# KhutornoyYaroslav/vcm-ts

Hardware: AMD Instinct MI355X
Metric: encoded frames/sec at 1920x1080 GOP-32 (higher is better)
Workload: dtype f32 (fp16x3 split-MFMA, fp32 accumulate)

## Files before the change

### include/dcvc_hip.h

```cpp
#ifndef DCVC_HIP_H
#define DCVC_HIP_H

#include <stdint.h>

#ifdef __cplusplus
extern "C" {
#endif

#define DCVC_OK 0
#define DCVC_E_ARG (-1)
#define DCVC_E_LAUNCH (-2)
#define DCVC_E_RANGE (-3)

#define DCVC_STATUS_ACT_SATURATED 1

#define DCVC_MAX_SEG 3

#define DCVC_PREC_FP32 0
#define DCVC_PREC_FP16X3 1

typedef struct {
    const float *ptr;
    int32_t C;
    int32_t cs;
// ... 1 lines not shown

typedef struct {
    dcvc_seg seg[DCVC_MAX_SEG];
    int32_t nseg;
    int32_t N, Hin, Win;
    int32_t in_act;
    float in_slope;
    const float *wpack;
    const float *bpack;
    int32_t ks;
    int32_t stride;
    int32_t Cout;
    int32_t Cout_pad;
    float *out;
    int32_t out_cs;
    int32_t out_act;
    float out_slope;
    int32_t pixel_shuffle;
    const float *res;
    int32_t res_cs;
    const float *res_gate;
    const float *res2;
    int32_t res2_cs;
    int32_t precision;
    int32_t *status;
    float *chan_partial;
    int32_t tile_row0;
    int32_t tile_rows;
    int32_t pair_taps;
} dcvc_conv_args;

int32_t dcvc_conv_tile_rows(int32_t ks, int32_t stride);

int32_t dcvc_conv_chan_partial_parts(int32_t ks, int32_t stride, int32_t Hout, int32_t Wout);
int dcvc_channel_mean_finish(const float *chan_partial, int32_t parts, int32_t row_stride, float *mean, int32_t N,
                             int32_t C, int32_t HW, void *stream);

int64_t dcvc_conv_pack_size(int32_t Cout, int32_t ks, int32_t nseg, const int32_t *seg_C, int32_t *cout_pad);

int dcvc_conv_pack_weights(const float *w, const float *b, int32_t Cout, int32_t ks, int32_t nseg,
                           const int32_t *seg_C, int32_t pixel_shuffle, int32_t precision, float *wpack,
                           float *bpack);

int64_t dcvc_conv_pack_size_paired(int32_t Cout, int32_t Cin, int32_t *cout_pad);
int dcvc_conv_pack_weights_paired(const float *w, const float *b, int32_t Cout, int32_t Cin, float *wpack, float *bpack);

int dcvc_conv2d(const dcvc_conv_args *a, void *stream);
int dcvc_conv_set_lookahead(int32_t mode);

int64_t dcvc_conv_small_pack_bytes(int32_t Cout, int32_t ks, int32_t nseg, const int32_t *seg_C);
int dcvc_conv_small_pack_weights(const float *w, const float *b, int32_t Cout, int32_t ks, int32_t nseg,
                                 const int32_t *seg_C, void *wpack, float *bpack);
int dcvc_conv2d_small(const dcvc_conv_args *a, void *stream);

int64_t dcvc_conv_k32_pack_bytes(int32_t Cout, int32_t ks, int32_t nseg, const int32_t *seg_C, int32_t *cout_pad);
int dcvc_conv_k32_pack_weights(const float *w, const float *b, int32_t Cout, int32_t ks, int32_t nseg,
                               const int32_t *seg_C, int32_t pixel_shuffle, void *wpack, float *bpack);
int dcvc_conv2d_k32(const dcvc_conv_args *a, void *stream);
int dcvc_conv_k32_set_waves(int32_t waves);

int dcvc_warp(const float *src, int32_t src_cs, const float *flow, int32_t flow_cs, float *out, int32_t out_cs,
              int32_t N, int32_t H, int32_t W, int32_t C, void *stream);
int dcvc_up2(const float *src, int32_t src_cs, float *out, int32_t out_cs, float *out2, int32_t out2_cs,
             int32_t N, int32_t H, int32_t W, int32_t C, float scale, void *stream);
int dcvc_down2(const float *src, int32_t src_cs, float *out, int32_t out_cs, int32_t N, int32_t H, int32_t W,
               int32_t C, float scale, int32_t avgpool_order, void *stream);
int dcvc_maxpool2(const float *src, int32_t src_cs, float *out, int32_t out_cs, int32_t N, int32_t H, int32_t W,
                  int32_t C, void *stream);
int dcvc_copy_channels(const float *src, int32_t src_cs, float *out, int32_t out_cs, int64_t npix, int32_t C,
                       void *stream);
int dcvc_nchw_to_nhwc(const float *src, float *out, int32_t out_cs, int32_t N, int32_t C, int32_t H, int32_t W,
                      void *stream);
int dcvc_nhwc_to_nchw(const float *src, int32_t src_cs, float *out, int32_t N, int32_t C, int32_t H, int32_t W,
                      int32_t clamp01, void *stream);

int dcvc_channel_mean(const float *src, int32_t src_cs, float *mean, float *scratch, int32_t N, int32_t HW,
                      int32_t C, void *stream);
int dcvc_se_gate(const float *mean, const float *w1, const float *w2, float *gate, int32_t N, int32_t C,
                 int32_t Cr, void *stream);

int dcvc_scale_channels(const float *src, int32_t src_cs, float *out, int32_t out_cs, const float *q_basic,
                        const float *q_scale, int32_t mode, int32_t N, int32_t HW, int32_t C, void *stream);
int dcvc_scale_channels_map(const float *src, int32_t src_cs, float *out, int32_t out_cs, const float *q_basic,
                            const float *q_scale, int32_t mode, int32_t N, int32_t HW, int32_t C, const float *q_map,
                            int32_t H, int32_t W, void *stream);
int dcvc_round_symbols(const float *z, int32_t z_cs, float *z_hat, int32_t zh_cs, int32_t *sym, int32_t N,
                       int32_t H, int32_t W, int32_t C, void *stream);
int dcvc_symbols_to_nhwc(const int32_t *sym, float *out, int32_t out_cs, int32_t N, int32_t H, int32_t W,
                         int32_t C, void *stream);

typedef struct {
    const float *y;
    int32_t y_cs;
    const float *fusion;
    int32_t fusion_cs;
    const float *spatial;
    int32_t spatial_cs;
    float *params;
    int32_t params_cs;
    float *y_hat;
    float *y_q;
    float *y_res;
    float *scales_hat;
    int32_t *sym;
    int32_t *idx;
    float *out;
// ... 35 lines not shown
```

### vcm_ts_amd/csrc/conv_small.hip

```cpp
#include <hip/hip_runtime.h>
#include <stdint.h>
#include <string.h>

#include "dcvc_hip.h"
#include "kernel_common.h"

namespace {

constexpr int KC = 16;

struct SmallK {
    const float *seg_ptr[DCVC_MAX_SEG];
    int seg_C[DCVC_MAX_SEG];
    int seg_cs[DCVC_MAX_SEG];
    int nseg;
    int H, W;
    int in_act;
    float in_slope;
    const char *wpack;
    const float *bpack;
    int Cout;
    float *out;
    int out_cs, out_act;
    float out_slope;
    const float *res;
    int res_cs;
    int *status;
};

template <int KS>
__global__ __launch_bounds__(256, 3) void conv_small(const SmallK a) {
    constexpr int RPW = 2, BH = 4 * RPW, BW = 32, PAD = KS / 2, PH = BH + KS - 1, PW = BW + KS - 1, T = KS * KS;
    constexpr int TPS = KS, NST = KS;
    constexpr int PATCH_F = PH * PW * 16;
    constexpr int SLAB_F = TPS * 4 * 16 * 4;
    __shared__ __attribute__((aligned(16))) float lds[PATCH_F + SLAB_F];
    char *patch = (char *)lds;
    float *wl = lds + PATCH_F;

    const int tid = threadIdx.x, lane = tid & 63, wave = tid >> 6;
    const int x0 = blockIdx.x * BW, y0 = blockIdx.y * BH, img = blockIdx.z;
    const int pr = lane & 15, g = lane >> 4;

    f32x4 acc[RPW][2];
#pragma unroll
    for (int m = 0; m < RPW; ++m)
#pragma unroll
        for (int hf = 0; hf < 2; ++hf) acc[m][hf] = (f32x4){0.f, 0.f, 0.f, 0.f};

    constexpr int NP = (PH * PW * 4 + 255) / 256, NW = (SLAB_F / 4 + 255) / 256;
    f32x4 rp[NP], rw[NW];
    struct Cursor {
        int s, c0, cg, st;
    };
    auto advance = [&](Cursor &k) {
// ... 85 lines not shown
        Cursor nxt = cur;
        advance(nxt);
        if (nxt.s < a.nseg) {
            if (nxt.st == 0) load_patch(nxt);
            load_w(nxt);
        }
#pragma unroll
        for (int tt = 0; tt < TPS; ++tt) {
            const f16x8 b1 = *(const f16x8 *)&wl[((tt * 4 + (g & 1)) * 16 + pr) * 4];
            const f16x8 b2 = g < 2 ? *(const f16x8 *)&wl[((tt * 4 + 2 + g) * 16 + pr) * 4] : zero8;
#pragma unroll
            for (int m = 0; m < RPW; ++m)
#pragma unroll
                for (int hf = 0; hf < 2; ++hf) {
                    const int p = (wave * RPW + m + cur.st) * PW + hf * 16 + pr + tt;
                    const f16x8 av = *(const f16x8 *)(patch + p * 64 + ((g ^ ((p >> 1) & 3)) << 4));
                    acc[m][hf] = __builtin_amdgcn_mfma_f32_16x16x32_f16(av, b1, acc[m][hf], 0, 0, 0);
                    acc[m][hf] = __builtin_amdgcn_mfma_f32_16x16x32_f16(av, b2, acc[m][hf], 0, 0, 0);
                }
        }
        cur = nxt;
    }

    const float inv_scale = 1.f / (ACT_SCALE * WGT_SCALE);
    const int ch = pr;
    bool sat = false;
    if (ch < a.Cout) {
        const float bias = a.bpack[ch];
#pragma unroll
        for (int m = 0; m < RPW; ++m) {
            const int oy = y0 + wave * RPW + m;
            if (oy >= a.H) continue;
            float rv[2][4];
#pragma unroll
            for (int hf = 0; hf < 2; ++hf)
#pragma unroll
                for (int j = 0; j < 4; ++j) {
                    const int ox = x0 + hf * 16 + g * 4 + j;
                    rv[hf][j] = (a.res && ox < a.W) ? a.res[((size_t)(img * a.H + oy) * a.W + ox) * a.res_cs + ch] : 0.f;
                }
#pragma unroll
            for (int hf = 0; hf < 2; ++hf)
#pragma unroll
                for (int j = 0; j < 4; ++j) {
                    const int ox = x0 + hf * 16 + g * 4 + j;
                    if (ox >= a.W) continue;
                    float v = acc[m][hf][j] * inv_scale + bias;
                    if (a.out_act == 1) v = act(v, a.out_slope);
                    else if (a.out_act == 2) v = fminf(fmaxf(v, 0.f), 1.f);
                    if (a.res) v += rv[hf][j];
                    if (a.status && !(fabsf(v) <= ACT_LIMIT)) sat = true;
                    a.out[((size_t)(img * a.H + oy) * a.W + ox) * a.out_cs + ch] = v;
                }
        }
    }
    if (sat) atomicOr(a.status, DCVC_STATUS_ACT_SATURATED);
}

}

extern "C" int64_t dcvc_conv_small_pack_bytes(int32_t Cout, int32_t ks, int32_t nseg, const int32_t *seg_C) {
    if (Cout <= 0 || Cout > 16 || nseg <= 0 || nseg > DCVC_MAX_SEG || (ks != 3 && ks != 7)) return DCVC_E_ARG;
    int chunks = 0;
    for (int s = 0; s < nseg; ++s) {
        if (seg_C[s] <= 0) return DCVC_E_ARG;
        chunks += (seg_C[s] + KC - 1) / KC;
    }
    return (int64_t)chunks * ks * ks * 1024;
}

extern "C" int dcvc_conv_small_pack_weights(const float *w, const float *b, int32_t Cout, int32_t ks, int32_t nseg,
                                            const int32_t *seg_C, void *wpack, float *bpack) {
    const int64_t total = dcvc_conv_small_pack_bytes(Cout, ks, nseg, seg_C);
    if (total < 0 || !w || !wpack || !bpack) return DCVC_E_ARG;
    const int T = ks * ks;
    int Cin = 0;
    for (int s = 0; s < nseg; ++s) Cin += seg_C[s];
    memset(wpack, 0, (size_t)total);
    for (int n = 0; n < 16; ++n) bpack[n] = (b && n < Cout) ? b[n] : 0.f;
    _Float16 *base = (_Float16 *)wpack;
    int status = DCVC_OK, cg = 0, cin0 = 0;
    for (int s = 0; s < nseg; ++s) {
        for (int c0 = 0; c0 < seg_C[s]; c0 += KC, ++cg)
            for (int t = 0; t < T; ++t)
                for (int cc = 0; cc < KC && c0 + cc < seg_C[s]; ++cc)
                    for (int n = 0; n < Cout; ++n) {
                        float sv = w[((size_t)n * Cin + cin0 + c0 + cc) * T + t] * WGT_SCALE;
                        if (!(fabsf(sv) <= F16_MAX)) { status = DCVC_E_RANGE; sv = sv > 0.f ? F16_MAX : -F16_MAX; }
                        const SplitF16 p = split_f16(sv);
                        const size_t blk = ((size_t)cg * T + t) * 4;
                        base[((blk + (cc >> 3)) * 16 + n) * 8 + (cc & 7)] = p.hi;
                        base[((blk + 2 + (cc >> 3)) * 16 + n) * 8 + (cc & 7)] = p.lo;
                    }
        cin0 += seg_C[s];
    }
    return status;
}

extern "C" int dcvc_conv2d_small(const dcvc_conv_args *a, void *stream) {
    if (!conv_args_ok(a)) return DCVC_E_ARG;
    if (a->out_act < 0 || a->out_act > 2) return DCVC_E_ARG;
    if (a->tile_rows > 0) return DCVC_E_ARG;
    if (a->Cout <= 0 || a->Cout > 16 || (a->ks != 3 && a->ks != 7) || a->stride != 1 || a->pixel_shuffle || a->res_gate ||
        a->res2 || a->chan_partial || a->precision != DCVC_PREC_FP16X3 || a->N <= 0)
        return DCVC_E_ARG;
    SmallK k;
    memset(&k, 0, sizeof(k));
    copy_conv_args(k, a);
    k.H = a->Hin, k.W = a->Win;
    dim3 grid((unsigned)((a->Win + 31) / 32), (unsigned)((a->Hin + 7) / 8), (unsigned)a->N);
    if (a->ks == 7)
        hipLaunchKernelGGL(conv_small<7>, grid, dim3(256), 0, (hipStream_t)stream, k);
    else
        hipLaunchKernelGGL(conv_small<3>, grid, dim3(256), 0, (hipStream_t)stream, k);
    RET_LAUNCH();
}
```

### vcm_ts_amd/engine.py

```python
from __future__ import annotations

import ctypes as C
import math

import numpy as np
import torch

from . import lib

_raw_stream = getattr(torch._C, "_cuda_getCurrentRawStream", None) or (lambda idx: torch.cuda.current_stream(idx).cuda_stream)


def _r4(c):
    return (c + 3) // 4 * 4


class View:

    __slots__ = ("base", "N", "H", "W", "C", "cs", "coff", "ptr")

    def __init__(self, base: torch.Tensor, C_: int, coff: int = 0, geom=None):
        self.base = base
        if geom is None:
            assert base.dim() == 4 and base.dtype == torch.float32 and base.is_contiguous()
            self.N, self.H, self.W, self.cs = base.shape
            self.ptr = base.data_ptr() + 4 * coff
        else:
            self.N, self.H, self.W, self.cs, self.ptr = geom
        self.C = C_
        self.coff = coff
        assert coff + C_ <= self.cs

    @staticmethod
    def alias(t: torch.Tensor):
        if t.dim() != 4 or t.dtype != torch.float32 or not t.is_cuda:
            return None
        N, C_, H, W = t.shape
        cs = t.stride(3)
        if t.stride(1) == 1 and cs >= C_ and cs % 4 == 0 and t.stride(2) == W * cs and t.stride(0) == H * W * cs \
                and t.data_ptr() % 16 == 0:
            return View(t, C_, 0, geom=(N, H, W, cs, t.data_ptr()))
        return None

    def slice(self, c0: int, c: int) -> "View":
        v = View(self.base, c, 0, geom=(self.N, self.H, self.W, self.cs, self.ptr + 4 * c0))
        v.coff = self.coff + c0
        return v

    def nchw(self) -> torch.Tensor:
        if self.base.dim() == 4 and tuple(self.base.shape) == (self.N, self.H, self.W, self.cs):
            return self.base[..., self.coff : self.coff + self.C].permute(0, 3, 1, 2)
        return self.base[:, self.coff : self.coff + self.C]

    @property
    def HW(self):
        return self.H * self.W

    def __repr__(self):
        return f"View(N={self.N},H={self.H},W={self.W},C={self.C},cs={self.cs},coff={self.coff})"


class PackedConv:
    __slots__ = ("w", "b", "ks", "Cout", "Cout_pad", "seg_C", "ps", "version", "precision", "weight", "bias",
                 "cin_slice", "key", "small", "k32", "paired", "host", "job")


class Engine:
    def __init__(self, device, precision=None):
        import os

        self.precision = precision or os.environ.get("DCVC_PRECISION", "fp32")
        if self.precision not in lib.PRECISIONS:
            raise ValueError(f"precision must be one of {sorted(lib.PRECISIONS)}")
        self.device = torch.device(device)
        if self.device.type != "cuda":
            raise RuntimeError("the HIP engine needs a GPU device (no CPU fallback exists)")
        self._dev_index = self.device.index if self.device.index is not None else torch.cuda.current_device()
        self.L = lib.hip()
        self.bufs = {}
        self.packs = {}
        self._dev_packs = []
        self._plan = None
        self.calls = 0
        self.profile = None
        self.profile_detail = None
        self.profile_hbm = None
        self.tape = None
        self._edges = {}
        self._status = None
        dev = os.environ.get("DCVC_DEV") == "1"
        sw = lambda name, default: os.environ.get(name, default) if dev else default
        self.use_small = sw("DCVC_SMALL", "1") != "0"
        self.use_k32 = sw("DCVC_K32", "1") != "0"
        self.use_pairs = sw("DCVC_PAIR_TAPS", "1") != "0"
        self.k32_everywhere = False
        self.k32_sizes = tuple(int(k) for k in sw("DCVC_K32_SIZES", "3").split(","))
        self.range_check = os.environ.get("DCVC_RANGE_CHECK", "1") == "1"
        self.guard_outputs = True
        self.wgrad_split = os.environ.get("DCVC_WGRAD_SPLIT", "1") != "0"
        self.wgrad_side_stream = sw("DCVC_WGRAD_SIDE", "1") != "0"

    def stream(self):
        return C.c_void_p(_raw_stream(self._dev_index))

    def _store(self, scratch=False):
        return self.bufs if (self.tape is None or scratch) else self.tape.arena

    def buf(self, name, N, H, W, C_, cs=None, zero=False) -> View:
        cs = cs or _r4(C_)
        key = (name, N, H, W, cs)
        store = self._store()
        t = store.get(key)
        if t is None:
            t = (torch.zeros if zero else torch.empty)((N, H, W, cs), dtype=torch.float32, device=self.device)
            store[key] = t
        return View(t, C_)

    def status_word(self) -> torch.Tensor:
        if self._status is None:
            self._status = torch.zeros(1, dtype=torch.int32, device=self.device)
        return self._status

    def read_status(self) -> int:
        if self._status is None:
            return 0
        v = int(self._status.item())
        if v:
            self._status.zero_()
        return v

    def check_status(self):
        self._raise_if_clamped(0 if self._status is None else int(self._status.item()))

    def _raise_if_clamped(self, v):
        if v:
            self._status.zero_()
            raise lib.KernelError(f"split-fp16 activation range exceeded (status {v}): |x| > 8188; use precision='fp32'")

    def status_snapshot(self):
        if self._status is None:
            return None
        host = torch.empty(1, dtype=torch.int32, pin_memory=True)
        host.copy_(self._status, non_blocking=True)
        ev = torch.cuda.Event()
        ev.record(torch.cuda.current_stream(self.device))
# ... 97 lines not shown
            pk.precision = lib.PRECISIONS[self.precision]
            pk.key = key
            self.packs[key] = pk
            self._dev_packs.append(pk)
        assert weight.is_contiguous() and weight.dtype == torch.float32 and weight.device == self.device
        segs = (C.c_int32 * len(seg_C))(*seg_C)
        lib.check(self.L.dcvc_conv_pack_weights_dev(weight.data_ptr(), None if (bias is None or transposed) else bias.data_ptr(),
                                                    Cout, CinT, ks, len(seg_C), segs, off, int(ps), pk.precision,
                                                    int(transposed), pk.w.data_ptr(), pk.b.data_ptr(), self.stream()),
                  f"conv_pack_weights_dev({key})")
        pk.version = ver
        pk.weight, pk.bias, pk.cin_slice = weight, bias, cin_slice
        pk.job = (weight, None if (bias is None or transposed) else bias, Cout, CinT, ks, tuple(seg_C), off, int(ps),
                  int(transposed))
        return pk

    def repack_all(self):
        packs = self._dev_packs
        if len(packs) < 8:
            return
        vers, stale = [], False
        for pk in packs:
            w, b = pk.job[0], pk.job[1]
            ver = (w._version, None if pk.bias is None else pk.bias._version, w.data_ptr())
            stale = stale or pk.version != ver
            vers.append(ver)
        if not stale:
            return
        ptrs = tuple(v[2] for v in vers)
        if self._plan is None or self._plan[1] != len(packs) or self._plan[2] != ptrs:
            if self._plan is not None:
                self.L.dcvc_pack_plan_destroy(self._plan[0])
                self._plan = None
            jobs = (lib.PackJob * len(packs))()
            for j, pk in zip(jobs, packs):
                w, b, Cout, CinT, ks, seg_C, off, ps, transposed = pk.job
                j.w, j.b = w.data_ptr(), None if b is None else b.data_ptr()
                j.Cout, j.Cin_total, j.ks, j.nseg = Cout, CinT, ks, len(seg_C)
                for i, c in enumerate(seg_C):
                    j.seg_C[i] = c
                j.cin_offset, j.pixel_shuffle, j.precision, j.transposed = off, ps, pk.precision, transposed
                j.wpack, j.bpack = pk.w.data_ptr(), pk.b.data_ptr()
            handle = C.c_void_p()
            torch.cuda.synchronize(self.device)
            lib.check(self.L.dcvc_pack_plan_create(jobs, len(packs), C.byref(handle)), "pack_plan_create")
            self._plan = (handle, len(packs), ptrs)
        lib.check(self.L.dcvc_pack_plan_run(self._plan[0], self.stream()), "pack_plan_run")
        for pk, ver in zip(packs, vers):
            pk.version = ver

    _HOST_PACKINGS = {
        "mfma": ("dcvc_conv_pack_size", 4, "dcvc_conv_pack_weights", ("ps", "precision"), None),
        "small": ("dcvc_conv_small_pack_bytes", 1, "dcvc_conv_small_pack_weights", (), 16),
        "paired": ("dcvc_conv_pack_size_paired", 4, "dcvc_conv_pack_weights_paired", (), None),
        "k32": ("dcvc_conv_k32_pack_bytes", 1, "dcvc_conv_k32_pack_weights", ("ps",), None),
    }

    def _pack_host(self, variant, key, weight, bias, seg_C, ps, cin_slice, ver) -> PackedConv:
        size_fn, unit, pack_fn, extra, cpad_fixed = self._HOST_PACKINGS[variant]
        w = weight.detach().float().cpu()
        if cin_slice is not None:
            w = w[:, cin_slice[0] : cin_slice[1]]
        w = w.contiguous().numpy()
        Cout, Cin, ks, _ = w.shape
        assert sum(seg_C) == Cin, (key, seg_C, Cin)
        if self.precision == "fp16x3" and not np.isfinite(w).all():
            raise lib.KernelError(f"{pack_fn[5:]}({key}): {int((~np.isfinite(w)).sum())} non-finite weight(s) cannot be "
                                  f"represented in split fp16, use precision='fp32'")
        b = None if bias is None else bias.detach().float().cpu().contiguous().numpy()
        segs = (C.c_int32 * len(seg_C))(*seg_C)
        layer = (Cout, Cin) if variant == "paired" else (Cout, ks, len(seg_C), segs)
        cpad = C.c_int32(cpad_fixed or 0)
        n = getattr(self.L, size_fn)(*layer, *(() if cpad_fixed else (C.byref(cpad),)))
        if n < 0:
            raise lib.KernelError(f"{size_fn[5:]}({key})")
        wp = np.empty(n * unit // 4, np.float32)
        bp = np.empty(cpad.value, np.float32)
        opts = {"ps": int(ps), "precision": lib.PRECISIONS[self.precision]}
        lib.check(getattr(self.L, pack_fn)(w.ctypes.data, None if b is None else b.ctypes.data, *layer,
                                           *(opts[k] for k in extra), wp.ctypes.data, bp.ctypes.data),
                  f"{pack_fn[5:]}({key}) [status -3: a |weight| >= 1023.5 does not fit split fp16, use precision='fp32']")
        pk = PackedConv()
        pk.w, pk.b = torch.from_numpy(wp).to(self.device), torch.from_numpy(bp).to(self.device)
        pk.ks, pk.Cout, pk.Cout_pad, pk.seg_C, pk.ps, pk.version = ks, Cout, cpad.value, tuple(seg_C), bool(ps) and "ps" in extra, ver
        pk.precision = opts["precision"]
        pk.weight, pk.bias, pk.cin_slice, pk.key = weight, bias, cin_slice, key
        return pk

    def pack(self, key, weight: torch.Tensor, bias, seg_C, ps, cin_slice=None) -> PackedConv:
        if self.tape is not None:
            return self.pack_dev(key, weight, bias, seg_C, ps, cin_slice)
        ver = (weight._version, None if bias is None else bias._version, weight.data_ptr())
        key = (key, self.precision)
        pk = self.packs.get(key)
        if pk is None or pk.version != ver:
            pk = self.packs[key] = self._pack_host("mfma", key, weight, bias, seg_C, ps, cin_slice, ver)
            pk.host = True
        return pk

    def _repacked(self, pk: PackedConv, variant) -> PackedConv:
        q = getattr(pk, variant, None)
        if q is None or q.version != pk.version:
            q = self._pack_host(variant, pk.key, pk.weight, pk.bias, pk.seg_C, pk.ps, pk.cin_slice, pk.version)
            setattr(pk, variant, q)
        return q

    def pair_capable(self, pk: PackedConv, stride) -> bool:
        return (self.precision == "fp16x3" and self.tape is None and self.use_pairs and getattr(pk, "host", False)
                and pk.ks == 7 and stride == 1 and len(pk.seg_C) == 1 and pk.seg_C[0] <= 8 and not pk.ps and pk.Cout > 16)

    def k32_capable(self, pk: PackedConv, stride, out: View, res, res2, gate, srcs=()) -> bool:
        if not (self.precision == "fp16x3" and self.tape is None and self.use_k32 and getattr(pk, "host", False)):
            return False
        cfin = pk.Cout // 4 if pk.ps else pk.Cout
        al = lambda v: v is None or (v.ptr % 16 == 0 and v.cs % 4 == 0)
        covered = (pk.ks in self.k32_sizes and stride == 1 and all(c % 32 == 0 for c in pk.seg_C) and cfin % 4 == 0
                   and al(out) and al(res) and al(res2) and (gate is None or gate.data_ptr() % 16 == 0)
                   and all(al(s) for s in srcs) and out.H * out.W < (1 << 24)
                   and all(v is None or v.cs * 4 < (1 << 24) for v in (out, res, res2, *srcs)))
        if not covered or self.k32_everywhere:
            return covered
        m = 2 if pk.ps else 1
        tiles = ((out.H // m + 7) // 8) * ((out.W // m + 31) // 32)
        return pk.Cout_pad % 64 == 0 and tiles * (pk.Cout_pad // 64) >= 1000

    def small_capable(self, pk: PackedConv, stride, gate, res2, chan_partial) -> bool:
        return (self.precision == "fp16x3" and self.tape is None and self.use_small and getattr(pk, "host", False)
                and pk.Cout <= 16 and pk.ks in (3, 7)
                and stride == 1 and not pk.ps and gate is None and res2 is None and chan_partial is None)

    def conv(self, pk: PackedConv, srcs, out: View, stride=1, in_slope=None, out_slope=None, res: View = None,
             gate: torch.Tensor = None, res2: View = None, chan_partial: torch.Tensor = None, band=None):
        return self._conv_f32(pk, srcs, out, stride, in_slope, out_slope, res, gate, res2, chan_partial, band)

    def _launch_conv(self, launch, pk, s0, Ho, Wo, stride, res, res2, tag="", note=""):
        if self.profile is None:
            launch()
            return
        ev0, ev1 = self._bracket(launch)
        flops = 2.0 * s0.N * Ho * Wo * pk.Cout * sum(pk.seg_C) * pk.ks * pk.ks
        nout = s0.N * Ho * Wo * pk.Cout
        abytes = 4.0 * (s0.N * s0.H * s0.W * sum(pk.seg_C) + nout * (1 + (res is not None) + (res2 is not None))
                        + pk.Cout * sum(pk.seg_C) * pk.ks * pk.ks)
        self.profile.setdefault(f"conv{pk.ks}x{pk.ks}s{stride}{tag}", []).append((ev0, ev1, flops, abytes))
        if self.profile_detail is not None:
            self.profile_detail.append((ev0, ev1, flops, f"k{pk.ks}s{stride}{tag} {pk.seg_C}->{pk.Cout}{'ps' if pk.ps else ''} "
                                                         f"{s0.H}x{s0.W}", note))

    @staticmethod
    def _bracket(launch):
        ev0, ev1 = torch.cuda.Event(enable_timing=True), torch.cuda.Event(enable_timing=True)
        ev0.record()
        launch()
        ev1.record()
        return ev0, ev1

    def chan_partial_buf(self, name, pk: PackedConv, out: View, stride=1):
        parts = int(self.L.dcvc_conv_chan_partial_parts(pk.ks, stride, out.H, out.W))
        if parts <= 0:
            raise lib.KernelError("conv_chan_partial_parts")
        return self.fbuf(name + ".chan_partial", out.N * parts * pk.Cout_pad), parts

    def _conv_f32(self, pk: PackedConv, srcs, out: View, stride=1, in_slope=None, out_slope=None, res: View = None,
                  gate: torch.Tensor = None, res2: View = None, chan_partial: torch.Tensor = None, band=None):
        a = lib.ConvArgs()
        assert len(srcs) == len(pk.seg_C)
        s0 = srcs[0]
        for i, (s, c) in enumerate(zip(srcs, pk.seg_C)):
            assert s.C == c and (s.N, s.H, s.W) == (s0.N, s0.H, s0.W), (s, c)
            a.seg[i].ptr, a.seg[i].C, a.seg[i].cs = s.ptr, s.C, s.cs
        a.nseg, a.N, a.Hin, a.Win = len(srcs), s0.N, s0.H, s0.W
        a.in_act, a.in_slope = (0, 0.0) if in_slope is None else (1, in_slope)
        small = band is None and self.small_capable(pk, stride, gate, res2, chan_partial)
        k32 = not small and not isinstance(out_slope, tuple) and self.k32_capable(pk, stride, out, res, res2, gate, srcs)
        paired = not small and not k32 and self.pair_capable(pk, stride)
        wq = self._repacked(pk, "small" if small else ("k32" if k32 else "paired")) if (small or k32 or paired) else pk
        a.pair_taps = int(paired)
        a.wpack, a.bpack = wq.w.data_ptr(), wq.b.data_ptr()
        a.ks, a.stride, a.Cout, a.Cout_pad = pk.ks, stride, pk.Cout, wq.Cout_pad
        pad = pk.ks // 2
        Ho = (s0.H + 2 * pad - pk.ks) // stride + 1
        Wo = (s0.W + 2 * pad - pk.ks) // stride + 1
        m = 2 if pk.ps else 1
        cfin = pk.Cout // 4 if pk.ps else pk.Cout
        assert (out.N, out.H, out.W, out.C) == (s0.N, Ho * m, Wo * m, cfin), (out, Ho, Wo, cfin)
        a.out, a.out_cs = out.ptr, out.cs
        if isinstance(out_slope, tuple):
            assert out_slope[0] == "mask" and res2 is not None and not (small or k32)
            a.out_act, a.out_slope = 3, float(out_slope[1])
        else:
            a.out_act, a.out_slope = (0, 0.0) if out_slope is None else ((2, 0.0) if out_slope == "clamp01" else (1, out_slope))
        a.pixel_shuffle = int(pk.ps)
        a.precision = pk.precision
        if res is not None:
            assert (res.N, res.H, res.W, res.C) == (out.N, out.H, out.W, out.C)
            a.res, a.res_cs = res.ptr, res.cs
        if gate is not None:
            a.res_gate = gate.data_ptr()
        if res2 is not None:
            assert (res2.N, res2.H, res2.W, res2.C) == (out.N, out.H, out.W, out.C)
            a.res2, a.res2_cs = res2.ptr, res2.cs
        if (self.range_check or k32) and self.precision == "fp16x3" and self.guard_outputs:
            a.status = self.status_word().data_ptr()
        if chan_partial is not None:
            a.chan_partial = chan_partial.data_ptr()
        if band is not None:
            a.tile_row0, a.tile_rows = int(band[0]), int(band[1])
        fn, what = (self.L.dcvc_conv2d_small, "conv2d_small") if small else (
            (self.L.dcvc_conv2d_k32, "conv2d_k32") if k32 else (self.L.dcvc_conv2d, "conv2d"))
        note = ""
        if self.profile_detail is not None:
            note = (f"{pk.key[0][1] if isinstance(pk.key[0], tuple) and len(pk.key[0]) > 1 else pk.key[0]}"
                    f" in_act={in_slope} out_act={out_slope} in_cs={[s.cs for s in srcs]} out_cs={out.cs}"
                    f" res={None if res is None else res.cs} gate={gate is not None} res2={None if res2 is None else res2.cs}"
                    f" chan_sums={chan_partial is not None}")
        self._launch_conv(lambda: lib.check(fn(C.byref(a), self.stream()), what), pk, s0, Ho, Wo, stride, res, res2,
                          "small" if small else ("k32" if k32 else ""), note)
        self.calls += 1
        self._rec("conv", pk, tuple(srcs), out, stride, in_slope, out_slope, res, gate, res2)
        return out

    def _hbm(self, kernel, shape, abytes, launch):
        if self.profile_hbm is None:
            return launch()
        ev0, ev1 = self._bracket(launch)
        self.profile_hbm.setdefault((kernel, shape), []).append((ev0, ev1, float(abytes)))

    def collect_profile_hbm(self):
        torch.cuda.synchronize(self.device)
        out = []
        for (kernel, shape), v in (self.profile_hbm or {}).items():
            ms = sum(r[0].elapsed_time(r[1]) for r in v)
            by = sum(r[2] for r in v)
            out.append({"kernel": kernel, "shape": shape, "launches": len(v), "avg_us": round(ms / len(v) * 1e3, 2),
                        "algorithmic_bytes": int(by / len(v)), "tb_per_s": round(by / (ms * 1e-3) / 1e12, 3) if ms > 0 else None})
        return out

    def collect_profile(self):
        torch.cuda.synchronize(self.device)
        return {k: {"flops": sum(r[2] for r in v), "bytes": sum(r[3] for r in v),
                    "ms": sum(r[0].elapsed_time(r[1]) for r in v), "launches": len(v)}
                for k, v in (self.profile or {}).items()}

    def warp(self, src: View, flow: View, out: View):
        self._hbm("warp", f"C{src.C} {src.H}x{src.W}", src.N * src.H * src.W * (8 * src.C + 8),
                  lambda: lib.check(self.L.dcvc_warp(src.ptr, src.cs, flow.ptr, flow.cs, out.ptr, out.cs, src.N, src.H, src.W,
                                                     src.C, self.stream()), "warp"))
        self.calls += 1
        self._rec("warp", src, flow, out)
        return out

    def up2(self, src: View, out: View, scale=1.0, out2: View = None):
        n_in = src.N * src.H * src.W * src.C * 4
        self._hbm("up2", f"C{src.C} {src.H}x{src.W}", n_in * (1 + 4 * (2 if out2 else 1)),
                  lambda: lib.check(self.L.dcvc_up2(src.ptr, src.cs, out.ptr, out.cs, out2.ptr if out2 else None,
                                                    out2.cs if out2 else 0, src.N, src.H, src.W, src.C, scale, self.stream()), "up2"))
        self.calls += 1
        self._rec("up2", src, out, scale, out2)
        return out

    def down2(self, src: View, out: View, scale=1.0, avgpool_order=False):
# ... 141 lines not shown
```

### vcm_ts_amd/lib.py

```python
from __future__ import annotations

import ctypes as C
import functools
import os

HERE = os.path.dirname(os.path.abspath(__file__))
CSRC = os.path.join(HERE, "csrc")


class LibraryMissing(RuntimeError):
    pass


class KernelError(RuntimeError):
    pass


def _load(name):
    path = os.environ.get("DCVC_HIP_LIB") if name == "libdcvc_hip.so" and os.environ.get("DCVC_HIP_LIB") else \
        os.path.join(CSRC, name)
    if not os.path.exists(path):
        raise LibraryMissing(f"{path} not built; run `make -C {CSRC}` (no CPU fallback exists)")
    return C.CDLL(path)

# ... 71 lines not shown

class PackJob(C.Structure):
    _fields_ = [
        ("w", C.c_void_p), ("b", C.c_void_p), ("Cout", C.c_int32), ("Cin_total", C.c_int32), ("ks", C.c_int32),
        ("nseg", C.c_int32), ("seg_C", C.c_int32 * 3), ("cin_offset", C.c_int32), ("pixel_shuffle", C.c_int32),
        ("precision", C.c_int32), ("transposed", C.c_int32), ("wpack", C.c_void_p), ("bpack", C.c_void_p),
    ]


class DualPriorBwdArgs(C.Structure):
    _fields_ = [
        ("y", C.c_void_p), ("y_cs", C.c_int32), ("fusion", C.c_void_p), ("fusion_cs", C.c_int32),
        ("y_hat", C.c_void_p), ("dout", C.c_void_p), ("dout_cs", C.c_int32), ("dy_res", C.c_void_p),
        ("dscales_hat", C.c_void_p), ("dparams", C.c_void_p), ("dparams_cs", C.c_int32),
        ("dspatial", C.c_void_p), ("dspatial_cs", C.c_int32), ("dy", C.c_void_p), ("dy_cs", C.c_int32),
        ("dfusion", C.c_void_p), ("dfusion_cs", C.c_int32), ("dq_plane", C.c_void_p),
        ("q_basic", C.c_void_p), ("q_scale", C.c_void_p), ("N", C.c_int32), ("H", C.c_int32), ("W", C.c_int32),
        ("C", C.c_int32), ("step", C.c_int32),
    ]


class ColorCoeffs(C.Structure):
    _fields_ = [(n, C.c_float) for n in ("y_off", "c_off", "y_scale", "c_scale", "crr", "cgb", "cgr", "cbb", "kr", "kg", "kb",
                                         "icb", "icr", "y_range", "c_range")] + \
               [(n, C.c_int32) for n in ("max_code", "bit_depth", "siting", "matrix", "range")]


class RoiBox(C.Structure):
    _fields_ = [(n, C.c_int32) for n in ("x1", "y1", "x2", "y2", "cls")]


class RoiClassRec(C.Structure):
    _fields_ = [("border", C.c_int32), ("shrink", C.c_int32), ("feather", C.c_float * 64)]


PRECISIONS = {"fp32": 0, "fp16x3": 1}

i32, i64, f32, vp = C.c_int32, C.c_int64, C.c_float, C.c_void_p

HEADERS = {
    "dcvc_hip.h": {
        "dcvc_conv_tile_rows": (i32, i32, i32),
        "dcvc_conv_chan_partial_parts": (i32, i32, i32, i32, i32),
        "dcvc_channel_mean_finish": [vp, i32, i32, vp, i32, i32, i32, vp],
        "dcvc_conv_pack_size": (i64, i32, i32, i32, vp, C.POINTER(i32)),
        "dcvc_conv_pack_weights": [vp, vp, i32, i32, i32, vp, i32, i32, vp, vp],
        "dcvc_conv_pack_size_paired": (i64, i32, i32, C.POINTER(i32)),
        "dcvc_conv_pack_weights_paired": [vp, vp, i32, i32, vp, vp],
        "dcvc_conv2d": [C.POINTER(ConvArgs), vp],
        "dcvc_conv_set_lookahead": [i32],
        "dcvc_conv_small_pack_bytes": (i64, i32, i32, i32, vp),
        "dcvc_conv_small_pack_weights": [vp, vp, i32, i32, i32, vp, vp, vp],
        "dcvc_conv2d_small": [C.POINTER(ConvArgs), vp],
        "dcvc_conv_k32_pack_bytes": (i64, i32, i32, i32, vp, C.POINTER(i32)),
        "dcvc_conv_k32_pack_weights": [vp, vp, i32, i32, i32, vp, i32, vp, vp],
        "dcvc_conv2d_k32": [C.POINTER(ConvArgs), vp],
        "dcvc_conv_k32_set_waves": [i32],
        "dcvc_warp": [vp, i32, vp, i32, vp, i32, i32, i32, i32, i32, vp],
        "dcvc_up2": [vp, i32, vp, i32, vp, i32, i32, i32, i32, i32, f32, vp],
        "dcvc_down2": [vp, i32, vp, i32, i32, i32, i32, i32, f32, i32, vp],
        "dcvc_maxpool2": [vp, i32, vp, i32, i32, i32, i32, i32, vp],
        "dcvc_copy_channels": [vp, i32, vp, i32, i64, i32, vp],
        "dcvc_nchw_to_nhwc": [vp, vp, i32, i32, i32, i32, i32, vp],
        "dcvc_nhwc_to_nchw": [vp, i32, vp, i32, i32, i32, i32, i32, vp],
        "dcvc_channel_mean": [vp, i32, vp, vp, i32, i32, i32, vp],
        "dcvc_se_gate": [vp, vp, vp, vp, i32, i32, i32, vp],
        "dcvc_scale_channels": [vp, i32, vp, i32, vp, vp, i32, i32, i32, i32, vp],
        "dcvc_scale_channels_map": [vp, i32, vp, i32, vp, vp, i32, i32, i32, i32, vp, i32, i32, vp],
        "dcvc_round_symbols": [vp, i32, vp, i32, vp, i32, i32, i32, i32, vp],
        "dcvc_symbols_to_nhwc": [vp, vp, i32, i32, i32, i32, i32, vp],
        "dcvc_scale_indexes": [vp, vp, i64, vp, vp],
        "dcvc_dual_prior_enc": [C.POINTER(DualPriorArgs), vp],
        "dcvc_dual_prior_dec_index": [C.POINTER(DualPriorArgs), vp],
        "dcvc_dual_prior_dec_apply": [C.POINTER(DualPriorArgs), vp],
        "dcvc_scale_bits": [vp, vp, vp, vp, i32, i32, i64, vp],
        "dcvc_factorized_bits": [vp, i32, vp, vp, vp, i32, i32, i32, vp],
        "dcvc_sq_err": [vp, i32, vp, i32, vp, vp, i32, i32, i32, vp],
        "dcvc_cdf_table_cols": (i32,),
        "dcvc_build_scale_cdfs": [vp, i32, i32, vp, vp, vp, vp],
        "dcvc_build_factorized_cdfs": [vp, i32, vp, vp, vp, vp],
        "dcvc_hip_version": (C.c_char_p,),
    },
    "dcvc_hip_grad.h": {
        "dcvc_conv_pack_weights_dev": [vp, vp, i32, i32, i32, i32, vp, i32, i32, i32, i32, vp, vp, vp],
        "dcvc_pack_plan_create": [C.POINTER(PackJob), i32, C.POINTER(C.c_void_p)],
        "dcvc_pack_plan_run": [vp, vp],
        "dcvc_pack_plan_destroy": (None, vp),
        "dcvc_conv_bwd_prologue": [C.POINTER(ConvBwdArgs), vp],
        "dcvc_conv_wgrad_scratch_min": (i64, i32, i32, i32),
        "dcvc_conv_wgrad": [C.POINTER(WgradArgs), vp],
        "dcvc_channel_dot": [vp, i32, vp, i32, vp, vp, i32, i32, i32, i32, i32, vp],
        "dcvc_mask_accumulate": [vp, i32, vp, i32, f32, vp, i32, i64, i32, vp],
        "dcvc_add_planes": [vp, i32, vp, i32, vp, i32, i64, i32, vp],
        "dcvc_warp_bwd": [vp, i32, vp, i32, vp, i32, vp, i32, vp, i32, i32, i32, i32, i32, vp, vp],
        "dcvc_up2_bwd": [vp, i32, vp, i32, i32, i32, i32, i32, f32, vp],
        "dcvc_down2_bwd": [vp, i32, vp, i32, i32, i32, i32, i32, f32, vp],
        "dcvc_maxpool2_bwd": [vp, i32, vp, i32, vp, i32, i32, i32, i32, i32, vp],
        "dcvc_se_bwd": [vp, vp, vp, vp, vp, vp, vp, vp, i32, i32, i32, vp],
        "dcvc_add_channel_vec": [vp, i32, vp, f32, i32, i32, i32, vp],
        "dcvc_scale_channels_bwd": [vp, i32, vp, i32, vp, vp, i32, i32, i32, i32, vp],
        "dcvc_q_finish": [vp, vp, vp, vp, vp, vp, i32, i32, vp],
        "dcvc_dual_prior_bwd": [C.POINTER(DualPriorBwdArgs), vp],
        "dcvc_scale_bits_bwd": [vp, vp, vp, vp, vp, i32, i32, i64, vp],
        "dcvc_factorized_bits_bwd": [vp, i32, vp, vp, vp, i32, vp, i32, i32, i32, vp],
        "dcvc_sq_err_bwd": [vp, i32, vp, i32, vp, vp, i32, i32, i32, i32, vp],
    },
# ... 118 lines not shown
```

Measured before the change: 42.62.

## Add phase-packed MFMA kernel for tiny-Cout convs packing J pixels per N-column

Adds a new conv kernel for convolutions with Cout<=4 (ks 3 or 7, stride 1). It packs J horizontally adjacent output pixels into the 16 MFMA output columns by replicating shifted weight copies, so the tensor-core tile is not mostly wasted on padding channels. Weights get a new phase-packed layout, and the input patch is staged in LDS with a phase-interleaved, swizzled layout. The cost is more weight data and more MFMAs per tap (KS+J-1 shifted slots), plus a new code path that is enabled by default.

```diff
diff --git a/include/dcvc_hip.h b/include/dcvc_hip.h
--- a/include/dcvc_hip.h
+++ b/include/dcvc_hip.h
@@ -77,6 +77,11 @@
 int dcvc_conv_small_pack_weights(const float *w, const float *b, int32_t Cout, int32_t ks, int32_t nseg,
                                  const int32_t *seg_C, void *wpack, float *bpack);
 int dcvc_conv2d_small(const dcvc_conv_args *a, void *stream);
+
+int64_t dcvc_conv_phase_pack_bytes(int32_t Cout, int32_t ks, int32_t nseg, const int32_t *seg_C);
+int dcvc_conv_phase_pack_weights(const float *w, const float *b, int32_t Cout, int32_t ks, int32_t nseg,
+                                 const int32_t *seg_C, void *wpack, float *bpack);
+int dcvc_conv2d_phase(const dcvc_conv_args *a, void *stream);
 
 int64_t dcvc_conv_k32_pack_bytes(int32_t Cout, int32_t ks, int32_t nseg, const int32_t *seg_C, int32_t *cout_pad);
 int dcvc_conv_k32_pack_weights(const float *w, const float *b, int32_t Cout, int32_t ks, int32_t nseg,
diff --git a/vcm_ts_amd/csrc/conv_small.hip b/vcm_ts_amd/csrc/conv_small.hip
--- a/vcm_ts_amd/csrc/conv_small.hip
+++ b/vcm_ts_amd/csrc/conv_small.hip
@@ -1,6 +1,8 @@
 #include <hip/hip_runtime.h>
 #include <stdint.h>
 #include <string.h>
+
+#include <type_traits>
 
 #include "dcvc_hip.h"
 #include "kernel_common.h"
@@ -192,6 +194,204 @@
                     if (a.status && !(fabsf(v) <= ACT_LIMIT)) sat = true;
                     a.out[((size_t)(img * a.H + oy) * a.W + ox) * a.out_cs + ch] = v;
                 }
+        }
+    }
+    if (sat) atomicOr(a.status, DCVC_STATUS_ACT_SATURATED);
+}
+
+
+constexpr int phase_j(int Cout) { return Cout <= 2 ? 8 : (Cout <= 4 ? 4 : 0); }
+
+template <int KS, int J>
+__global__ __launch_bounds__(256) void conv_small_phase(const SmallK a) {
+    constexpr int NWV = 4, NT = 64 * NWV, MT = 4 / NWV, BH = 8, GX = 8, BW = GX * J, PAD = KS / 2, PH = BH + KS - 1, PW = BW + KS - 1;
+    constexpr int CP = 16 / J, NS = KS + J - 1;
+    constexpr int NG = (PW + J - 1) / J, RS = NG * J;
+    constexpr int NREC = PH * RS;
+    constexpr int PATCH_F = NREC * 16;
+    constexpr int TAPB = CP * 16, ROWB = ((J - 1 + KS) * TAPB + 255) / 256 * 256, WL_B = KS * 4 * ROWB + 256;
+    static_assert((J - 1) * TAPB <= 256, "the last row's overrun stays inside the array");
+    __shared__ __attribute__((aligned(16))) float lds[PATCH_F + WL_B / 4];
+    char *patch = (char *)lds;
+    char *wl = (char *)(lds + PATCH_F);
+
+    const int tid = threadIdx.x, lane = tid & 63, wave = tid >> 6;
+    const int x0 = blockIdx.x * BW, y0 = blockIdx.y * BH, img = blockIdx.z;
+    const int pr = lane & 15, g = lane >> 4;
+
+    f32x4 acc[MT];
+#pragma unroll
+    for (int m = 0; m < MT; ++m) acc[m] = (f32x4){0.f, 0.f, 0.f, 0.f};
+
+    constexpr int NE = KS * 4 * KS * CP;
+    constexpr int NP = (NREC * 4 + NT - 1) / NT, NW = (NE + NT - 1) / NT;
+    f32x4 rp[NP], rw[NW];
+    struct Cursor {
+        int s, c0, cg;
+    };
+    static_assert(NP <= 32, "one bit per staged float4");
+    auto pixel_of = [&](int t, int u) {
+        const int i = t + u * NT;
+        const int rec = i >> 2;
+        const int py = rec / RS, rem = rec - py * RS;
+        const int ph = rem / NG, px = (rem - ph * NG) * J + ph;
+        const int gy = y0 - PAD + py, gx = x0 - PAD + px;
+        const bool ok = (i < NREC * 4) & (px < PW) & ((unsigned)gy < (unsigned)a.H) & ((unsigned)gx < (unsigned)a.W);
+        return ok ? gy * a.W + gx : -1;
+    };
+    unsigned inpic = 0;
+#pragma unroll
+    for (int u = 0; u < NP; ++u) inpic |= (pixel_of(tid, u) >= 0 ? 1u : 0u) << u;
+    auto load_patch = [&](const Cursor &k) {
+        const int C = a.seg_C[k.s], cs = a.seg_cs[k.s];
+        const float *sp = a.seg_ptr[k.s] + (size_t)img * a.H * a.W * cs;
+        const int c = k.c0 + (tid & 3) * 4;
+        const int cc = c < C ? c : 0;
+        int t = tid;
+        asm volatile("" : "+v"(t));
+#pragma unroll
+        for (int u = 0; u < NP; ++u) {
+            const int p = pixel_of(t, u);
+            rp[u] = *(const f32x4 *)(sp + (size_t)(p < 0 ? 0 : p) * cs + cc);
+        }
+    };
+    auto store_patch = [&](const Cursor &k) {
+        const int C = a.seg_C[k.s];
+#pragma unroll
+        for (int u = 0; u < NP; ++u) {
+            const int i = tid + u * NT;
+            if (i < NREC * 4) {
+                const int qd = i & 3, rec = i >> 2;
+                const int c = k.c0 + qd * 4;
+                f32x4 v = ((inpic >> u) & 1u) && c < C ? rp[u] : (f32x4){0.f, 0.f, 0.f, 0.f};
+                if (c + 3 >= C) {
+                    if (c + 1 >= C) v[1] = 0.f;
+                    if (c + 2 >= C) v[2] = 0.f;
+                    v[3] = 0.f;
+                }
+                if (a.in_act) {
+#pragma unroll
+                    for (int e = 0; e < 4; ++e) v[e] = act(v[e], a.in_slope);
+                }
+                f32x4 sv = v * ACT_SCALE;
+#pragma unroll
+                for (int e = 0; e < 4; ++e) sv[e] = __builtin_amdgcn_fmed3f(sv[e], -F16_MAX, F16_MAX);
+                const f16x4 hi = __builtin_convertvector(sv, f16x4);
+                const f16x4 lo = __builtin_convertvector(sv - __builtin_convertvector(hi, f32x4), f16x4);
+                const int sw = ((rec / RS) & 1) << 1, h = qd >> 1;
+                char *r = patch + rec * 64 + (qd & 1) * 8;
+                *(f16x4 *)(r + ((h ^ sw) << 4)) = hi;
+                *(f16x4 *)(r + (((2 + h) ^ sw) << 4)) = lo;
+            }
+        }
+    };
+    int wsrc[NW], wdst[NW];
+#pragma unroll
+    for (int u = 0; u < NW; ++u) {
+        const int e = (u + 1) * NT <= NE ? tid + u * NT : min(tid + u * NT, NE - 1);
+        const int ch = e % CP, kx = e / CP % KS, slot = e / (CP * KS) % 4, ky = e / (CP * KS * 4);
+        wsrc[u] = ((ky * NS + kx) * 4 + slot) * 256 + ch * 16;
+        wdst[u] = (ky * 4 + slot) * ROWB + (J - 1 + kx) * TAPB + ch * 16;
+    }
+    auto load_w = [&](const Cursor &k) {
+        const char *src = a.wpack + (size_t)k.cg * (KS * NS * 1024);
+#pragma unroll
+        for (int u = 0; u < NW; ++u) rw[u] = *(const f32x4 *)(src + wsrc[u]);
+    };
+    auto store_w = [&]() {
+#pragma unroll
+        for (int u = 0; u < NW; ++u) *(f32x4 *)(wl + wdst[u]) = rw[u];
+    };
+    for (int i = tid; i < WL_B / 16; i += NT) *(f32x4 *)(wl + i * 16) = (f32x4){0.f, 0.f, 0.f, 0.f};
+    auto following = [&](const Cursor &k) {
+        Cursor n = {k.s, k.c0 + KC, k.cg + 1};
+        if (n.c0 >= a.seg_C[n.s]) {
+            ++n.s;
+            n.c0 = 0;
+        }
+        return n;
+    };
+
+    const f16x8 zero8 = {0, 0, 0, 0, 0, 0, 0, 0};
+    const int arow = wave * MT * 2 + (pr >> 3), agx = pr & 7;
+    struct Frag {
+        f16x8 b1, b2, av[MT];
+    };
+    const char *abase[2], *b1base = wl + (g & 1) * ROWB + (J - 1 - pr / CP) * TAPB + (pr % CP) * 16, *b2base = b1base + 2 * ROWB;
+#pragma unroll
+    for (int par = 0; par < 2; ++par) abase[par] = patch + (arow * RS + agx) * 64 + ((g ^ (((arow + par) & 1) << 1)) << 4);
+    auto frag = [&](Frag &f, int ky, int s) {
+        f.b1 = *(const f16x8 *)(b1base + ky * 4 * ROWB + s * TAPB);
+        f.b2 = g < 2 ? *(const f16x8 *)(b2base + ky * 4 * ROWB + s * TAPB) : zero8;
+#pragma unroll
+        for (int m = 0; m < MT; ++m)
+            f.av[m] = *(const f16x8 *)(abase[ky & 1] + (((2 * m + ky) * RS) + (s % J) * NG + s / J) * 64);
+    };
+    auto chunk = [&](const Cursor &cur, const Cursor &nxt, auto more) {
+        constexpr bool MORE = decltype(more)::value;
+        __syncthreads();
+        store_w();
+        store_patch(cur);
+        __syncthreads();
+        if (MORE) {
+            load_w(nxt);
+            load_patch(nxt);
+        }
+        __builtin_amdgcn_sched_barrier(0);
+        Frag f[2];
+        frag(f[0], 0, 0);
+#pragma unroll
+        for (int t = 0; t < KS * NS; ++t) {
+            if (t + 1 < KS * NS) frag(f[(t + 1) & 1], (t + 1) / NS, (t + 1) % NS);
+            const Frag &c = f[t & 1];
+#pragma unroll
+            for (int m = 0; m < MT; ++m) acc[m] = __builtin_amdgcn_mfma_f32_16x16x32_f16(c.av[m], c.b1, acc[m], 0, 0, 0);
+#pragma unroll
+            for (int m = 0; m < MT; ++m) acc[m] = __builtin_amdgcn_mfma_f32_16x16x32_f16(c.av[m], c.b2, acc[m], 0, 0, 0);
+            __builtin_amdgcn_sched_barrier(0);
+        }
+    };
+
+    Cursor cur = {0, 0, 0};
+    load_w(cur);
+    load_patch(cur);
+    for (;;) {
+        const Cursor nxt = following(cur);
+        if (nxt.s < a.nseg) {
+            chunk(cur, nxt, std::true_type{});
+        } else {
+            chunk(cur, nxt, std::false_type{});
+            break;
+        }
+        cur = nxt;
+    }
+
+    const float inv_scale = 1.f / (ACT_SCALE * WGT_SCALE);
+    const int ch = pr % CP, j = pr / CP;
+    bool sat = false;
+    if (ch < a.Cout) {
+        const float bias = a.bpack[ch];
+#pragma unroll
+        for (int m = 0; m < MT; ++m) {
+            const int oy = y0 + (wave * MT + m) * 2 + (g >> 1);
+            if (oy >= a.H) continue;
+            float rv[4];
+#pragma unroll
+            for (int q = 0; q < 4; ++q) {
+                const int ox = x0 + ((g & 1) * 4 + q) * J + j;
+                rv[q] = (a.res && ox < a.W) ? a.res[((size_t)(img * a.H + oy) * a.W + ox) * a.res_cs + ch] : 0.f;
+            }
+#pragma unroll
+            for (int q = 0; q < 4; ++q) {
+                const int ox = x0 + ((g & 1) * 4 + q) * J + j;
+                if (ox >= a.W) continue;
+                float v = acc[m][q] * inv_scale + bias;
+                if (a.out_act == 1) v = act(v, a.out_slope);
+                else if (a.out_act == 2) v = fminf(fmaxf(v, 0.f), 1.f);
+                if (a.res) v += rv[q];
+                if (a.status && !(fabsf(v) <= ACT_LIMIT)) sat = true;
+                a.out[((size_t)(img * a.H + oy) * a.W + ox) * a.out_cs + ch] = v;
+            }
         }
     }
     if (sat) atomicOr(a.status, DCVC_STATUS_ACT_SATURATED);
@@ -255,3 +455,66 @@
         hipLaunchKernelGGL(conv_small<3>, grid, dim3(256), 0, (hipStream_t)stream, k);
     RET_LAUNCH();
 }
+
+extern "C" int64_t dcvc_conv_phase_pack_bytes(int32_t Cout, int32_t ks, int32_t nseg, const int32_t *seg_C) {
+    if (Cout <= 0 || phase_j(Cout) == 0 || nseg <= 0 || nseg > DCVC_MAX_SEG || !seg_C || (ks != 3 && ks != 7)) return DCVC_E_ARG;
+    int chunks = 0;
+    for (int s = 0; s < nseg; ++s) {
+        if (seg_C[s] <= 0) return DCVC_E_ARG;
+        chunks += (seg_C[s] + KC - 1) / KC;
+    }
+    return (int64_t)chunks * ks * (ks + phase_j(Cout) - 1) * 1024;
+}
+
+extern "C" int dcvc_conv_phase_pack_weights(const float *w, const float *b, int32_t Cout, int32_t ks, int32_t nseg,
+                                            const int32_t *seg_C, void *wpack, float *bpack) {
+    const int64_t total = dcvc_conv_phase_pack_bytes(Cout, ks, nseg, seg_C);
+    if (total < 0 || !w || !wpack || !bpack) return DCVC_E_ARG;
+    const int T = ks * ks, J = phase_j(Cout), CP = 16 / J, NS = ks + J - 1;
+    int Cin = 0;
+    for (int s = 0; s < nseg; ++s) Cin += seg_C[s];
+    memset(wpack, 0, (size_t)total);
+    for (int n = 0; n < 16; ++n) bpack[n] = (b && n < Cout) ? b[n] : 0.f;
+    _Float16 *base = (_Float16 *)wpack;
+    int status = DCVC_OK, cg = 0, cin0 = 0;
+    for (int s = 0; s < nseg; ++s) {
+        for (int c0 = 0; c0 < seg_C[s]; c0 += KC, ++cg)
+            for (int t = 0; t < T; ++t)
+                for (int cc = 0; cc < KC && c0 + cc < seg_C[s]; ++cc)
+                    for (int n = 0; n < Cout; ++n) {
+                        float sv = w[((size_t)n * Cin + cin0 + c0 + cc) * T + t] * WGT_SCALE;
+                        if (!(fabsf(sv) <= F16_MAX)) { status = DCVC_E_RANGE; sv = sv > 0.f ? F16_MAX : -F16_MAX; }
+                        const SplitF16 p = split_f16(sv);
+                        const int ky = t / ks, kx = t % ks;
+                        for (int j = 0; j < J; ++j) {
+                            const size_t blk = (((size_t)cg * ks + ky) * NS + kx + j) * 4;
+                            const int col = j * CP + n;
+                            base[((blk + (cc >> 3)) * 16 + col) * 8 + (cc & 7)] = p.hi;
+                            base[((blk + 2 + (cc >> 3)) * 16 + col) * 8 + (cc & 7)] = p.lo;
+                        }
+                    }
+        cin0 += seg_C[s];
+    }
+    return status;
+}
+
+extern "C" int dcvc_conv2d_phase(const dcvc_conv_args *a, void *stream) {
+    if (!conv_args_ok(a)) return DCVC_E_ARG;
+    if (a->out_act < 0 || a->out_act > 2) return DCVC_E_ARG;
+    if (a->tile_rows > 0) return DCVC_E_ARG;
+    if (a->Cout <= 0 || phase_j(a->Cout) == 0 || (a->ks != 3 && a->ks != 7) || a->stride != 1 || a->pixel_shuffle ||
+        a->res_gate || a->res2 || a->chan_partial || a->precision != DCVC_PREC_FP16X3 || a->N <= 0)
+        return DCVC_E_ARG;
+    SmallK k;
+    memset(&k, 0, sizeof(k));
+    copy_conv_args(k, a);
+    k.H = a->Hin, k.W = a->Win;
+    const int J = phase_j(a->Cout);
+    dim3 grid((unsigned)((a->Win + 8 * J - 1) / (8 * J)), (unsigned)((a->Hin + 7) / 8), (unsigned)a->N);
+    hipStream_t st = (hipStream_t)stream;
+    if (a->ks == 7 && J == 8) hipLaunchKernelGGL((conv_small_phase<7, 8>), grid, dim3(256), 0, st, k);
+    else if (a->ks == 7) hipLaunchKernelGGL((conv_small_phase<7, 4>), grid, dim3(256), 0, st, k);
+    else if (J == 8) hipLaunchKernelGGL((conv_small_phase<3, 8>), grid, dim3(256), 0, st, k);
+    else hipLaunchKernelGGL((conv_small_phase<3, 4>), grid, dim3(256), 0, st, k);
+    RET_LAUNCH();
+}
diff --git a/vcm_ts_amd/engine.py b/vcm_ts_amd/engine.py
--- a/vcm_ts_amd/engine.py
+++ b/vcm_ts_amd/engine.py
@@ -62,7 +62,7 @@
 
 class PackedConv:
     __slots__ = ("w", "b", "ks", "Cout", "Cout_pad", "seg_C", "ps", "version", "precision", "weight", "bias",
-                 "cin_slice", "key", "small", "k32", "paired", "host", "job")
+                 "cin_slice", "key", "small", "k32", "paired", "phase", "host", "job")
 
 
 class Engine:
@@ -91,6 +91,7 @@
         dev = os.environ.get("DCVC_DEV") == "1"
         sw = lambda name, default: os.environ.get(name, default) if dev else default
         self.use_small = sw("DCVC_SMALL", "1") != "0"
+        self.use_phase = sw("DCVC_PHASE", "1") != "0"
         self.use_k32 = sw("DCVC_K32", "1") != "0"
         self.use_pairs = sw("DCVC_PAIR_TAPS", "1") != "0"
         self.k32_everywhere = False
@@ -294,6 +295,7 @@
     _HOST_PACKINGS = {
         "mfma": ("dcvc_conv_pack_size", 4, "dcvc_conv_pack_weights", ("ps", "precision"), None),
         "small": ("dcvc_conv_small_pack_bytes", 1, "dcvc_conv_small_pack_weights", (), 16),
+        "phase": ("dcvc_conv_phase_pack_bytes", 1, "dcvc_conv_phase_pack_weights", (), 16),
         "paired": ("dcvc_conv_pack_size_paired", 4, "dcvc_conv_pack_weights_paired", (), None),
         "k32": ("dcvc_conv_k32_pack_bytes", 1, "dcvc_conv_k32_pack_weights", ("ps",), None),
     }
@@ -371,6 +373,12 @@
                 and pk.Cout <= 16 and pk.ks in (3, 7)
                 and stride == 1 and not pk.ps and gate is None and res2 is None and chan_partial is None)
 
+    PHASE_MAX_COUT = 4
+
+    def phase_capable(self, pk: PackedConv, stride, gate, res2, chan_partial) -> bool:
+        return (self.use_phase and self.small_capable(pk, stride, gate, res2, chan_partial)
+                and pk.Cout <= self.PHASE_MAX_COUT)
+
     def conv(self, pk: PackedConv, srcs, out: View, stride=1, in_slope=None, out_slope=None, res: View = None,
              gate: torch.Tensor = None, res2: View = None, chan_partial: torch.Tensor = None, band=None):
         return self._conv_f32(pk, srcs, out, stride, in_slope, out_slope, res, gate, res2, chan_partial, band)
@@ -414,9 +422,10 @@
         a.nseg, a.N, a.Hin, a.Win = len(srcs), s0.N, s0.H, s0.W
         a.in_act, a.in_slope = (0, 0.0) if in_slope is None else (1, in_slope)
         small = band is None and self.small_capable(pk, stride, gate, res2, chan_partial)
+        phase = small and self.phase_capable(pk, stride, gate, res2, chan_partial)
         k32 = not small and not isinstance(out_slope, tuple) and self.k32_capable(pk, stride, out, res, res2, gate, srcs)
         paired = not small and not k32 and self.pair_capable(pk, stride)
-        wq = self._repacked(pk, "small" if small else ("k32" if k32 else "paired")) if (small or k32 or paired) else pk
+        wq = self._repacked(pk, "phase" if phase else ("small" if small else ("k32" if k32 else "paired"))) if (small or k32 or paired) else pk
         a.pair_taps = int(paired)
         a.wpack, a.bpack = wq.w.data_ptr(), wq.b.data_ptr()
         a.ks, a.stride, a.Cout, a.Cout_pad = pk.ks, stride, pk.Cout, wq.Cout_pad
@@ -448,7 +457,7 @@
             a.chan_partial = chan_partial.data_ptr()
         if band is not None:
             a.tile_row0, a.tile_rows = int(band[0]), int(band[1])
-        fn, what = (self.L.dcvc_conv2d_small, "conv2d_small") if small else (
+        fn, what = (self.L.dcvc_conv2d_phase, "conv2d_phase") if phase else (self.L.dcvc_conv2d_small, "conv2d_small") if small else (
             (self.L.dcvc_conv2d_k32, "conv2d_k32") if k32 else (self.L.dcvc_conv2d, "conv2d"))
         note = ""
         if self.profile_detail is not None:
diff --git a/vcm_ts_amd/lib.py b/vcm_ts_amd/lib.py
--- a/vcm_ts_amd/lib.py
+++ b/vcm_ts_amd/lib.py
@@ -147,6 +147,9 @@
         "dcvc_conv_small_pack_bytes": (i64, i32, i32, i32, vp),
         "dcvc_conv_small_pack_weights": [vp, vp, i32, i32, i32, vp, vp, vp],
         "dcvc_conv2d_small": [C.POINTER(ConvArgs), vp],
+        "dcvc_conv_phase_pack_bytes": (i64, i32, i32, i32, vp),
+        "dcvc_conv_phase_pack_weights": [vp, vp, i32, i32, i32, vp, vp, vp],
+        "dcvc_conv2d_phase": [C.POINTER(ConvArgs), vp],
         "dcvc_conv_k32_pack_bytes": (i64, i32, i32, i32, vp, C.POINTER(i32)),
         "dcvc_conv_k32_pack_weights": [vp, vp, i32, i32, i32, vp, i32, vp, vp],
         "dcvc_conv2d_k32": [C.POINTER(ConvArgs), vp],
```

Result: no change. 42.99 (median of 6 runs) (+0.8%).
